# jyf588/transformer-inertial-poser

Measured on AMD Instinct MI355X. Metric: IMU frames/sec (whole node), seq_len=40 batch=256/GPU, higher is better.
Workload: dtype f32

## Files before the change

transformer-inertial-poser_amd/csrc/tip_attention.h:

```cpp
#pragma once
#include <hip/hip_runtime.h>

#include "tip_layernorm.h"

namespace tip {

typedef float f32x4_att __attribute__((ext_vector_type(4)));

template <int LDC, int LDV, bool DROP = false, int R0 = 0, int R1 = 3>
__device__ __forceinline__ void attention_head_mfma(float* Qc, float* Kc, const float* Vt, int c0, int lane, int row_limit = 48,
                                                    unsigned dkey = 0, unsigned thresh = 0, float dscale = 1.f,
                                                    unsigned long long bh = 0, int T = 0) {
    constexpr int RB = 3;
    const int l15 = lane & 15, lg = lane >> 4;
    float4 qf[RB], kf[RB];
#pragma unroll
    for (int r = 0; r < R1; ++r) {
        qf[r] = *reinterpret_cast<const float4*>(Qc + (r * 16 + l15) * LDC + c0 + lg * 4);
        kf[r] = *reinterpret_cast<const float4*>(Kc + (r * 16 + l15) * LDC + c0 + lg * 4);
    }
    f32x4_att S[RB][RB];
#pragma unroll
    for (int r = R0; r < R1; ++r)
#pragma unroll
// ... 66 lines not shown
        for (int e = 0; e < 4; ++e) {
            const float inv = __shfl(rsum[r], lg * 4 + e, 64);
            if (r * 16 + lg * 4 + e < row_limit) Qc[(r * 16 + lg * 4 + e) * LDC + c0 + l15] = o[e] * inv;
        }
    }
}

template <int LDC, bool TRAIN = false, bool STATS = true>
__device__ __forceinline__ void attention_head_regs(const f32x4_att (&qt)[3], const f32x4_att (&kt)[3], const f32x4_att (&v)[3],
                                                    float* Oc, int c0, int lane, int row_limit = 48, float* ast = nullptr,
                                                    unsigned long long bh = 0, int T = 0, unsigned long long seed = 0,
                                                    unsigned site = 0, unsigned thresh = 0, float dscale = 1.f) {
    constexpr int RB = 3;
    const int l15 = lane & 15, lg = lane >> 4;
    f32x4_att S[RB][RB];
#pragma unroll
    for (int r = 0; r < RB; ++r)
#pragma unroll
        for (int cb = 0; cb <= r; ++cb) {
            f32x4_att t = {0.f, 0.f, 0.f, 0.f};
#pragma unroll
            for (int e = 0; e < 4; ++e) t = __builtin_amdgcn_mfma_f32_16x16x4f32(kt[cb][e], qt[r][e], t, 0, 0, 0);
            S[r][cb] = t;
        }
    float mx[RB], rsum[RB];
#pragma unroll
    for (int r = 0; r < RB; ++r) {
        float m = -INFINITY;
#pragma unroll
        for (int e = 0; e < 4; ++e) {
            if (lg * 4 + e <= l15) m = fmaxf(m, S[r][r][e]);
#pragma unroll
            for (int cb = 0; cb < r; ++cb) m = fmaxf(m, S[r][cb][e]);
        }
        mx[r] = m;
    }
#pragma unroll
    for (int r = 0; r < RB; ++r) mx[r] = lg4_max(mx[r]);
#pragma unroll
    for (int r = 0; r < RB; ++r) {
        float sm = 0.f;
#pragma unroll
        for (int e = 0; e < 4; ++e) {
#pragma unroll
            for (int cb = 0; cb < r; ++cb) {
                const float p = __expf(S[r][cb][e] - mx[r]);
                S[r][cb][e] = p;
                sm += p;
            }
            const float pd = (lg * 4 + e <= l15) ? __expf(S[r][r][e] - mx[r]) : 0.f;
            S[r][r][e] = pd;
            sm += pd;
        }
        rsum[r] = sm;
    }
#pragma unroll
    for (int r = 0; r < RB; ++r) rsum[r] = lg4_sum(rsum[r]);
#pragma unroll
    for (int r = 0; r < RB; ++r) rsum[r] = 1.0f / rsum[r];
    if (TRAIN) {
        const unsigned dkey = tip_drop_key_s(seed, site);
        const __amdgpu_buffer_rsrc_t ars = tip_rows_buffer(ast + bh * T * 2, T * 8);
#pragma unroll
        for (int r = 0; r < RB; ++r) {
            const int q = r * 16 + l15;
            const ln_u32x2 mr = {__float_as_uint(mx[r]), __float_as_uint(rsum[r])};
            if (STATS) __builtin_amdgcn_raw_buffer_store_b64(mr, ars, lg == 0 ? q * 8 : T * 8, 0, 0);
            if (thresh) {
                const unsigned pb = (unsigned)((bh * T + q) * T);
#pragma unroll
                for (int cb = 0; cb <= r; ++cb)
#pragma unroll
                    for (int e = 0; e < 4; ++e)
                        S[r][cb][e] = tip_drop_hash_k(dkey, pb + cb * 16 + lg * 4 + e) >= thresh ? S[r][cb][e] * dscale : 0.f;
            }
        }
    }
#pragma unroll
    for (int r = 0; r < RB; ++r) {
        f32x4_att o = {0.f, 0.f, 0.f, 0.f};
#pragma unroll
        for (int kb = 0; kb <= r; ++kb)
#pragma unroll
            for (int e = 0; e < 4; ++e) o = __builtin_amdgcn_mfma_f32_16x16x4f32(S[r][kb][e], v[kb][e], o, 0, 0, 0);
#pragma unroll
        for (int e = 0; e < 4; ++e) {
            const float inv = __shfl(rsum[r], lg * 4 + e, 64);
            if (r * 16 + lg * 4 + e < row_limit) Oc[(r * 16 + lg * 4 + e) * LDC + c0 + l15] = o[e] * inv;
        }
    }
}

}
```

transformer-inertial-poser_amd/csrc/tip_fused.hip:

```cpp
#include <stdlib.h>
#include <string.h>

#include "tip_internal.h"
#include "tip_attention.h"
#include "tip_layernorm.h"

namespace tip {

typedef float f32x4 __attribute__((ext_vector_type(4)));

namespace fz {
constexpr int D = 256, H = 16, DH = 16, F = 1024, RP = 48, RB = 3, TMAX = 40, R = 512;
constexpr int KIN = 224;
constexpr int LDX = D + 8;
constexpr int LDC = 128 + 4;
constexpr int LDV = RP + 4;
constexpr int LDU = KIN + 8;
constexpr int X_FLOATS = RP * LDX;
constexpr int C_FLOATS = 2 * RP * LDC + 128 * LDV;
constexpr int LDS_BYTES = (X_FLOATS + C_FLOATS) * 4;
constexpr int THREADS = 512;
constexpr size_t IN_W = 0;
constexpr size_t IN_B = IN_W + (size_t)D * KIN;
constexpr size_t LAYER0 = IN_B + D;
// ... 65 lines not shown
        memcpy(L + G1, lw[8], sizeof(float) * D);
        memcpy(L + BE1, lw[9], sizeof(float) * D);
        memcpy(L + G2, lw[10], sizeof(float) * D);
        memcpy(L + BE2, lw[11], sizeof(float) * D);
    }
    if (fused_has_rnn_ih(d)) {
        const float* const* tw = t + 2 + 12 * d.L;
        float* I = dst + fused_ih_off(d);
        pack_frag(I, tw[0], R, D, D, nullptr, 1.f, 0);
        for (int i = 0; i < R; ++i) I[(size_t)R * D + i] = tw[2][i] + tw[3][i];
    }
}

static PackOp mk_op(const float* src, size_t dst, int N, int K, int src_rows, int src_cols, int frag) {
    PackOp o;
    o.src = src; o.src2 = nullptr; o.dst_off = dst; o.N = N; o.K = K; o.src_rows = src_rows; o.src_cols = src_cols; o.frag = frag;
    o.shuffle_h = 0; o.shuffle_dh = 0; o.z0 = 0; o.z1 = 0; o.scale_rows = 0; o.scale = 1.f; o.transpose = 0;
    return o;
}

void fused_pack_ops(const Dims& d, const float* const* t, size_t base, std::vector<PackOp>& ops) {
    using namespace fz;
    {
        PackOp o = mk_op(t[0], base + IN_W, D, KIN, D, d.In, 1);
        o.shuffle_h = H; o.shuffle_dh = DH;
        o.z0 = d.n_imu_total + d.rootv0; o.z1 = d.n_imu_total + d.rootv1;
        ops.push_back(o);
        PackOp b = mk_op(t[1], base + IN_B, D, 1, D, 1, 0);
        b.shuffle_h = H; b.shuffle_dh = DH;
        ops.push_back(b);
    }
    for (int l = 0; l < d.L; ++l) {
        const float* const* lw = t + 2 + 12 * l;
        const size_t L = base + LAYER0 + (size_t)l * LAYER_FLOATS;
        PackOp q = mk_op(lw[0], L + QKV_W, 3 * D, D, 3 * D, D, 1);
        q.scale = 0.25f; q.scale_rows = D;
        ops.push_back(q);
        PackOp qb = mk_op(lw[1], L + QKV_B, 3 * D, 1, 3 * D, 1, 0);
        qb.scale = 0.25f; qb.scale_rows = D;
        ops.push_back(qb);
        ops.push_back(mk_op(lw[2], L + WO_W, D, D, D, D, 1));
        ops.push_back(mk_op(lw[3], L + WO_B, D, 1, D, 1, 0));
        ops.push_back(mk_op(lw[4], L + W1_W, F, D, F, D, 1));
        ops.push_back(mk_op(lw[5], L + W1_B, F, 1, F, 1, 0));
        ops.push_back(mk_op(lw[6], L + W2_W, D, F, D, F, 1));
        ops.push_back(mk_op(lw[7], L + W2_B, D, 1, D, 1, 0));
        ops.push_back(mk_op(lw[8], L + G1, D, 1, D, 1, 0));
        ops.push_back(mk_op(lw[9], L + BE1, D, 1, D, 1, 0));
        ops.push_back(mk_op(lw[10], L + G2, D, 1, D, 1, 0));
        ops.push_back(mk_op(lw[11], L + BE2, D, 1, D, 1, 0));
    }
    if (fused_has_rnn_ih(d)) {
        const float* const* tw = t + 2 + 12 * d.L;
        const size_t I = base + fused_ih_off(d);
        ops.push_back(mk_op(tw[0], I, R, D, R, D, 1));
        PackOp b = mk_op(tw[2], I + (size_t)R * D, R, 1, R, 1, 0);
        b.src2 = tw[3];
        ops.push_back(b);
    }
}

__device__ __forceinline__ float wsum(float v) { return wave64_sum(v); }

template <int NBW, int SWAPN = 0>
__device__ __forceinline__ void mfma_block(f32x4 (&acc)[fz::RB][NBW], const float4 (&a)[fz::RB], const float4 (&w)[NBW]) {
#define TIP_MFMA_STEP(c)                                                                                             \
    _Pragma("unroll") for (int r = 0; r < fz::RB; ++r) _Pragma("unroll") for (int n = 0; n < NBW; ++n)                \
        acc[r][n] = n < SWAPN ? __builtin_amdgcn_mfma_f32_16x16x4f32(w[n].c, a[r].c, acc[r][n], 0, 0, 0)              \
                              : __builtin_amdgcn_mfma_f32_16x16x4f32(a[r].c, w[n].c, acc[r][n], 0, 0, 0);
    TIP_MFMA_STEP(x)
    TIP_MFMA_STEP(y)
    TIP_MFMA_STEP(z)
    TIP_MFMA_STEP(w)
#undef TIP_MFMA_STEP
}

typedef unsigned int u32x4 __attribute__((ext_vector_type(4)));

__device__ __forceinline__ float4 load_frag(__amdgpu_buffer_rsrc_t rsrc, int voff, int soff) {
    const f32x4 f = __builtin_bit_cast(f32x4, __builtin_amdgcn_raw_buffer_load_b128(rsrc, voff, soff, 0));
    return make_float4(f.x, f.y, f.z, f.w);
}

template <int NBW>
struct WRing {
    float4 w0[NBW], w1[NBW];
};

template <int NBW>
__device__ __forceinline__ void ring_prefetch(WRing<NBW>& g, __amdgpu_buffer_rsrc_t rsrc, int voff, int soff, int nstride_b) {
#pragma unroll
    for (int n = 0; n < NBW; ++n) {
        g.w0[n] = load_frag(rsrc, voff, soff + n * nstride_b);
        g.w1[n] = load_frag(rsrc, voff, soff + n * nstride_b + 1024);
    }
}

template <int NBW, int KB, bool NOMMA = false, int SWAPN = 0, bool PIN = true>
__device__ __forceinline__ void gemm_phase(f32x4 (&acc)[fz::RB][NBW], const float* As, int lda, __amdgpu_buffer_rsrc_t rsrc,
                                           int voff, int soff, int nstride_b, WRing<NBW>& g, int nsoff, int nnstride_b) {
    static_assert(KB % 2 == 0, "k-blocks are processed in pairs");
    float4 a0[fz::RB], a1[fz::RB];
#pragma unroll
    for (int r = 0; r < fz::RB; ++r) a0[r] = *reinterpret_cast<const float4*>(As + r * 16 * lda);
#pragma unroll 1
    for (int kb = 0; kb < KB; kb += 2) {
        const bool last = kb + 2 >= KB;
        const int o = last ? nsoff : soff + (kb + 2) * 1024;
        const int st = last ? nnstride_b : nstride_b;
#pragma unroll
        for (int r = 0; r < fz::RB; ++r) a1[r] = *reinterpret_cast<const float4*>(As + r * 16 * lda + (kb + 1) * 16);
        if (!NOMMA) mfma_block<NBW, SWAPN>(acc, a0, g.w0);
        else { asm volatile("" :: "v"(a0[0].x), "v"(g.w0[0].x)); }
#pragma unroll
        for (int n = 0; n < NBW; ++n) g.w0[n] = load_frag(rsrc, voff, o + n * st);
        if (PIN) __builtin_amdgcn_sched_barrier(0);
#pragma unroll
        for (int r = 0; r < fz::RB; ++r) a0[r] = *reinterpret_cast<const float4*>(As + r * 16 * lda + (kb + 2) * 16);
        if (!NOMMA) mfma_block<NBW, SWAPN>(acc, a1, g.w1);
        else { asm volatile("" :: "v"(a1[0].x), "v"(g.w1[0].x)); }
#pragma unroll
        for (int n = 0; n < NBW; ++n) g.w1[n] = load_frag(rsrc, voff, o + n * st + 1024);
        if (PIN) __builtin_amdgcn_sched_barrier(0);
    }
}

template <int NBW>
__device__ __forceinline__ void zero_acc(f32x4 (&acc)[fz::RB][NBW]) {
#pragma unroll
    for (int r = 0; r < fz::RB; ++r)
#pragma unroll
        for (int n = 0; n < NBW; ++n) acc[r][n] = (f32x4){0.f, 0.f, 0.f, 0.f};
}

__device__ __forceinline__ int opaque(int v) {
    asm volatile("" : "+v"(v));
    return v;
}

__device__ __forceinline__ void rows_to_hbm(const float* lds, int ld, int cols, float* dst, int dst_ld, int T, int tid) {
    const int c4n = cols >> 2;
    for (int i = tid; i < T * c4n; i += fz::THREADS) {
        const int r = i / c4n, c4 = i - r * c4n;
        __builtin_nontemporal_store(*reinterpret_cast<const f32x4*>(lds + r * ld + c4 * 4), reinterpret_cast<f32x4*>(dst + (size_t)r * dst_ld + c4 * 4));
    }
}

template <int COLS>
__device__ __forceinline__ void rows_to_hbm_fixed(const float* lds, int ld, float* dst, int dst_ld, int T, int tid) {
    constexpr int C4 = COLS / 4, NP = (40 * C4 + fz::THREADS - 1) / fz::THREADS;
    static_assert((NP * fz::THREADS + C4 - 1) / C4 <= fz::RP, "the passes stay inside the LDS tile's rows");
    const __amdgpu_buffer_rsrc_t rs = tip_rows_buffer(dst, T * dst_ld * 4);
#pragma unroll
    for (int j = 0; j < NP; ++j) {
        const int i = tid + j * fz::THREADS, r = i / C4, c4 = i - r * C4;
        const f32x4 v = *reinterpret_cast<const f32x4*>(lds + r * ld + c4 * 4);
        __builtin_amdgcn_raw_buffer_store_b128(__builtin_bit_cast(ln_u32x4, v), rs, (r * dst_ld + c4 * 4) * 4, 0, kTipNT);
    }
}

template <bool FIXED>
__device__ __forceinline__ void hidden_to_hbm(const float* lds, int ld, float* dst, int dst_ld, unsigned* gb, int f, int T, int tid) {
    typedef unsigned u32x4 __attribute__((ext_vector_type(4)));
    const int lane = tid & 63;
    if (FIXED) {
        const __amdgpu_buffer_rsrc_t rs = tip_rows_buffer(dst, T * dst_ld * 4);
// ... 438 lines not shown
    unsigned* __restrict__ hall_sentinel, int B, int T, int NI, int S, int L, int wbytes, int ih_off_b, FusedEncArgs<LIVE> tr) {
    using namespace fz;
    using namespace fzh;
    extern __shared__ __attribute__((aligned(16))) float smem[];
    float* X = smem;
    float* C = smem + X_FLOATS;
    const int tid = threadIdx.x, lane = tid & 63;
    const int wave = __builtin_amdgcn_readfirstlane(tid >> 6);
    const int l15 = lane & 15, lg = lane >> 4;
    const __amdgpu_buffer_rsrc_t rsrc = __builtin_amdgcn_make_buffer_rsrc(const_cast<float*>(wts), 0, wbytes, 0x00020000);
    const int voff = lane * 16;
    auto am = [&](int ld) { return l15 * ld + lg * 4; };
    auto at = [&](int ld) { return (TAIL0 + (lane & 3)) * ld + lg * 4; };
    constexpr bool DR = TR || LIVE;
    const LiveArgs lv = live_args_of(tr);
    unsigned long long dseed = tr.seed, sseed = 0;
    if (LIVE) {
        sseed = lv.state_seed;
        if (lv.seeds) { dseed = lv.seeds[0]; sseed = lv.seeds[1]; }
    }
    const unsigned mkey = LIVE && lv.mthresh ? tip_drop_key_s(sseed, kStateMaskSite) : 0u;

    for (int i = tid; i < 8 * LDX; i += THREADS) X[TMAX * LDX + i] = 0.f;

    for (int win = blockIdx.x; win < B; win += gridDim.x) {
        WRing<3> g_qkv;
        {
        const int layer = -1;
        FH_STAMP(0);
        if (TRACE && tid == 0 && win == (int)blockIdx.x && blockIdx.x < 1024) g_fh_wg[2 * blockIdx.x] = __builtin_amdgcn_s_memrealtime();
        const int in_soff = (int)(IN_W * 4) + (wave * 2) * (KIN / 16) * 1024;
        WRing<2> g_in;
        ring_prefetch<2>(g_in, rsrc, voff, in_soff, (KIN / 16) * 1024);
        float* U = C;
        for (int i = tid; i < RP * LDU / 4; i += THREADS) reinterpret_cast<float4*>(U)[i] = make_float4(0.f, 0.f, 0.f, 0.f);
        __syncthreads();
        {
            constexpr int NR = (TMAX + 7) / 8;
            float vi[NR][2], vs[NR][3], vk[NR][3];
            const float* kmb = keep_mask ? keep_mask : x_s;
#pragma unroll
            for (int j = 0; j < NR; ++j) {
                const int r = wave + 8 * j;
                const int rc = r < T ? r : T - 1;
                const float* xi = x_imu + ((size_t)win * T + rc) * NI;
                const float* xs = x_s + ((size_t)win * T + rc) * S;
                const float* km = kmb + ((size_t)win * T + rc) * S;
#pragma unroll
                for (int q = 0; q < 2; ++q) vi[j][q] = xi[lane + 64 * q < NI ? lane + 64 * q : NI - 1];
#pragma unroll
                for (int q = 0; q < 3; ++q) {
                    const int c = lane + 64 * q < S ? lane + 64 * q : S - 1;
                    vs[j][q] = xs[c];
                    vk[j][q] = km[c];
                }
            }
            float* pu_i = U + wave * LDU + lane;
            float* pu_s = pu_i + NI;
#pragma unroll
            for (int j = 0; j < NR; ++j) {
                if (wave + 8 * j < T) {
#pragma unroll
                    for (int q = 0; q < 2; ++q)
                        if (lane + 64 * q < NI) pu_i[8 * j * LDU + 64 * q] = vi[j][q];
#pragma unroll
                    for (int q = 0; q < 3; ++q)
                        if (lane + 64 * q < S) {
                            float v = vs[j][q];
                            if (v != v) v = 0.f;
                            if (keep_mask) v = v * vk[j][q] * keep_scale;
                            else if (LIVE && lv.mthresh)
                                v = v * (tip_drop_hash_k(mkey, ((unsigned)win * (unsigned)T + (unsigned)(wave + 8 * j)) * (unsigned)S + (unsigned)(lane + 64 * q)) >= lv.mthresh ? 1.f : 0.f) * keep_scale;
                            pu_s[8 * j * LDU + 64 * q] = v;
                        }
                }
            }
        }
        __syncthreads();
        FH_STAMP(1);
        if (TR && tr.u) rows_to_hbm_fixed<KIN>(U, LDU, tr.sv + (size_t)tr.u * 64 + (size_t)win * T * KIN, KIN, T, opaque(tid));
        {
            f32x4 acc[RBM][2], acct[RBT][2];
            zero_acc_h<2>(acc, acct);
            gemm_phase_h<2, KIN / 16, 0, TR>(acc, acct, U + am(LDU), U + at(LDU), LDU, rsrc, voff, in_soff, (KIN / 16) * 1024, g_in, in_soff,
                                      (KIN / 16) * 1024);
            ring_prefetch<3>(g_qkv, rsrc, voff, (int)(LAYER0 * 4) + (int)(QKV_W * 4) + wave * 16 * 1024, 16 * 16 * 1024);
#pragma unroll
            for (int n = 0; n < 2; ++n) {
                const int col = (wave * 2 + n) * 16 + l15;
                const float bv = wts[IN_B + col];
#pragma unroll
                for (int r = 0; r < RBM; ++r)
#pragma unroll
                    for (int e = 0; e < 4; ++e) X[(r * 16 + lg * 4 + e) * LDX + col] = acc[r][n][e] + bv;
#pragma unroll
                for (int r = 0; r < RBT; ++r) X[(TAIL0 + 4 * r + lg) * LDX + col] = tail_reduce(acct[r][n], lg) + bv;
            }
        }
        __syncthreads();
        FH_STAMP(2);
        }
        const size_t grow0 = (size_t)win * T;
        if (TR) rows_to_hbm_fixed<D>(X, LDX, tr.sv + (size_t)tr.x0 * 64 + grow0 * D, D, T, opaque(tid));
#pragma unroll 1
        for (int layer = 0; layer < L; ++layer) {
            FH_STAMP(8);
            const float* LW = wts + LAYER0 + (size_t)layer * LAYER_FLOATS;
            const int lbase = (int)((LAYER0 + (size_t)layer * LAYER_FLOATS) * 4);
            float* svl = TR ? tr.sv + (size_t)layer * tr.layer_stride * 64 : nullptr;
            const unsigned dk1 = DR ? tip_drop_key_s(dseed, (unsigned)(layer * 4 + 1)) : 0u;
            const unsigned dk2 = DR ? tip_drop_key_s(dseed, (unsigned)(layer * 4 + 2)) : 0u;
            const unsigned dk3 = DR ? tip_drop_key_s(dseed, (unsigned)(layer * 4 + 3)) : 0u;
            float bvo[2], bv2[2];
#pragma unroll
            for (int n = 0; n < 2; ++n) {
                bvo[n] = LW[WO_B + (wave * 2 + n) * 16 + l15];
                bv2[n] = LW[W2_B + (wave * 2 + n) * 16 + l15];
            }
            WRing<2> g_o, g_f;
            float* Oc = C;
#pragma unroll 1
            for (int c = 0; c < 2; ++c) {
                const int head = c * 8 + wave;
                f32x4 acc[RBM][3], acct[RBT][3];
                zero_acc_h<3>(acc, acct);
                const int qsoff = lbase + (int)(QKV_W * 4) + head * 16 * 1024;
                const int nxt = c == 0 ? qsoff + 8 * 16 * 1024 : qsoff;
                gemm_phase_h<3, 16, 2, TR>(acc, acct, X + am(LDX), X + at(LDX), LDX, rsrc, voff, qsoff, 16 * 16 * 1024, g_qkv, nxt,
                                       16 * 16 * 1024);
                if (c == 1)
                    ring_prefetch<2>(g_o, rsrc, voff, lbase + (int)(WO_W * 4) + (wave * 2) * 16 * 1024, 16 * 1024);
                const f32x4 bq = *reinterpret_cast<const f32x4*>(LW + QKV_B + head * 16 + lg * 4);
                const f32x4 bk = *reinterpret_cast<const f32x4*>(LW + QKV_B + D + head * 16 + lg * 4);
                const float bv = LW[QKV_B + 2 * D + head * 16 + l15];
                f32x4 qt[RB], kt[RB], vv[RB];
#pragma unroll
                for (int r = 0; r < RBM; ++r) {
                    qt[r] = acc[r][0] + bq;
                    kt[r] = acc[r][1] + bk;
                    vv[r] = acc[r][2] + bv;
                }
                vv[2] = tail_gather_v(acct[0][2], acct[1][2], lg);
                if (lg < 2) vv[2] += bv;
                {
                    constexpr int SLD = 20;
                    float* scr = C + RP * LDX + wave * (2 * 8 * SLD);
                    const float bqp = LW[QKV_B + head * 16 + l15], bkp = LW[QKV_B + D + head * 16 + l15];
#pragma unroll
                    for (int rb = 0; rb < RBT; ++rb) {
                        scr[(4 * rb + lg) * SLD + l15] = tail_reduce(acct[rb][0], lg) + bqp;
                        scr[8 * SLD + (4 * rb + lg) * SLD + l15] = tail_reduce(acct[rb][1], lg) + bkp;
                    }
                    __builtin_amdgcn_fence(__ATOMIC_RELEASE, "wavefront");
                    __builtin_amdgcn_wave_barrier();
                    __builtin_amdgcn_fence(__ATOMIC_ACQUIRE, "wavefront");
                    const f32x4 z = {0.f, 0.f, 0.f, 0.f};
                    qt[2] = l15 < 8 ? *reinterpret_cast<const f32x4*>(scr + l15 * SLD + lg * 4) : z;
                    kt[2] = l15 < 8 ? *reinterpret_cast<const f32x4*>(scr + 8 * SLD + l15 * SLD + lg * 4) : z;
                    __builtin_amdgcn_wave_barrier();
                }
                FH_STAMP(9 + 4 * c);
                if (TR) {
                    const __amdgpu_buffer_rsrc_t qp_rs = tip_rows_buffer(svl + (size_t)tr.qkv * 64 + grow0 * (3 * D), T * 3 * D * 4);
                    const int lo = opaque(lane), l15o = lo & 15, lgo = lo >> 4;
#pragma unroll
                    for (int r = 0; r < RB; ++r) {
                        const int qo = ((r * 16 + l15o) * (3 * D) + head * 16 + lgo * 4) * 4;
                        __builtin_amdgcn_raw_buffer_store_b128(__builtin_bit_cast(u32x4, qt[r] * 4.0f), qp_rs, qo, 0, kTipNT);
                        __builtin_amdgcn_raw_buffer_store_b128(__builtin_bit_cast(u32x4, kt[r]), qp_rs, qo + D * 4, 0, kTipNT);
#pragma unroll
                        for (int e = 0; e < 4; ++e)
                            __builtin_amdgcn_raw_buffer_store_b32(__float_as_uint(vv[r][e]), qp_rs,
                                                                  ((r * 16 + lgo * 4 + e) * (3 * D) + 2 * D + head * 16 + l15o) * 4, 0, kTipNT);
                    }
                    attention_head_regs<LDX, true>(qt, kt, vv, Oc, head * 16, lo, TMAX, svl + (size_t)tr.ast * 64,
                                                   (unsigned long long)win * H + head, T, tr.seed, (unsigned)(layer * 4 + 0), tr.thresh,
                                                   tr.scale);
                } else if (LIVE) {
                    attention_head_regs<LDX, true, false>(qt, kt, vv, Oc, head * 16, opaque(lane), TMAX, nullptr, (unsigned long long)win * H + head, T,
                                                          dseed, (unsigned)(layer * 4 + 0), tr.thresh, tr.scale);
                } else {
                    attention_head_regs<LDX>(qt, kt, vv, Oc, head * 16, lane, TMAX);
                }
                FH_STAMP(10 + 4 * c);
            }
            __syncthreads();
            FH_STAMP(15);
            if (TR) rows_to_hbm_fixed<D>(Oc, LDX, svl + (size_t)tr.att * 64 + grow0 * D, D, T, opaque(tid));
            ring_prefetch<2>(g_f, rsrc, voff, lbase + (int)(W1_W * 4) + (wave * 2) * 16 * 1024, 16 * 1024);
            f32x4 acc_o[RBM][2], acc_ot[RBT][2];
            zero_acc_h<2>(acc_o, acc_ot);
            {
                const int osoff = lbase + (int)(WO_W * 4) + (wave * 2) * 16 * 1024;
                gemm_phase_h<2, 16, 0, TR>(acc_o, acc_ot, Oc + am(LDX), Oc + at(LDX), LDX, rsrc, voff, osoff, 16 * 1024, g_o, osoff, 16 * 1024);
            }
            __syncthreads();
            FH_STAMP(16);
            float xr[2][RBM][4], xt[2][RBT];
#pragma unroll
            for (int n = 0; n < 2; ++n) {
                const int col = (wave * 2 + n) * 16 + l15;
#pragma unroll
                for (int r = 0; r < RBM; ++r)
#pragma unroll
                    for (int e = 0; e < 4; ++e) xr[n][r][e] = X[(r * 16 + lg * 4 + e) * LDX + col];
#pragma unroll
                for (int r = 0; r < RBT; ++r) xt[n][r] = X[(TAIL0 + 4 * r + lg) * LDX + col];
            }
#pragma unroll
            for (int n = 0; n < 2; ++n) {
                const int col = (wave * 2 + n) * 16 + l15;
                const float bv = bvo[n];
                    const int hl = LIVE ? opaque(lane) : lane, hlg = LIVE ? hl >> 4 : lg, hcol = LIVE ? (wave * 2 + n) * 16 + (hl & 15) : col;
#pragma unroll
                for (int r = 0; r < RBM; ++r)
#pragma unroll
                    for (int e = 0; e < 4; ++e) {
                        float v = acc_o[r][n][e] + bv;
                        if (DR && tr.thresh)
                            v = tip_drop_hash_k(dk1, (grow0 + r * 16 + hlg * 4 + e) * D + hcol) >= tr.thresh ? v * tr.scale : 0.f;
                        X[(r * 16 + lg * 4 + e) * LDX + col] = xr[n][r][e] + v;
                    }
#pragma unroll
                for (int r = 0; r < RBT; ++r) {
                    float v = tail_reduce(acc_ot[r][n], lg) + bv;
                    if (DR && tr.thresh)
                        v = tip_drop_hash_k(dk1, (grow0 + TAIL0 + 4 * r + hlg) * D + hcol) >= tr.thresh ? v * tr.scale : 0.f;
                    X[(TAIL0 + 4 * r + lg) * LDX + col] = xt[n][r] + v;
                }
            }
            __syncthreads();
            FH_STAMP(17);
            if (TR)
                layernorm_rows16<fz::TMAX, fz::LDX, true>(X, LW + G1, LW + BE1, wave, opaque(lane), svl + (size_t)tr.z1 * 64 + grow0 * D,
                                                          svl + (size_t)tr.st1 * 64 + grow0 * 2, svl + (size_t)tr.x1 * 64 + grow0 * D, T);
            else
                layernorm_rows16<fz::TMAX, fz::LDX>(X, LW + G1, LW + BE1, wave, lane);
            __syncthreads();
            FH_STAMP(18);
            float* Hc = C;
            f32x4 acc_f[RBM][2], acc_ft[RBT][2];
            zero_acc_h<2>(acc_f, acc_ft);
#pragma unroll 1
            for (int f = 0; f < 4; ++f) {
                {
                    f32x4 acc[RBM][2], acct[RBT][2];
                    zero_acc_h<2>(acc, acct);
                    const int nb0 = f * 16 + wave * 2;
                    const int w1off = lbase + (int)(W1_W * 4) + nb0 * 16 * 1024;
                    const int w2off = lbase + (int)(W2_W * 4) + ((wave * 2) * 64 + f * 16) * 1024;
                    float bv1[2];
#pragma unroll
                    for (int n = 0; n < 2; ++n) bv1[n] = LW[W1_B + f * 256 + (wave * 2 + n) * 16 + l15];
                    gemm_phase_h<2, 16, 0, TR>(acc, acct, X + am(LDX), X + at(LDX), LDX, rsrc, voff, w1off, 16 * 1024, g_f, w2off, 64 * 1024);
#pragma unroll
                    for (int n = 0; n < 2; ++n) {
                        const int col = (wave * 2 + n) * 16 + l15;
                        const float bv = bv1[n];
                    const int hl = LIVE ? opaque(lane) : lane, hlg = LIVE ? hl >> 4 : lg, hcol = LIVE ? (wave * 2 + n) * 16 + (hl & 15) : col;
#pragma unroll
                        for (int r = 0; r < RBM; ++r)
#pragma unroll
                            for (int e = 0; e < 4; ++e) {
                                float v = fmaxf(acc[r][n][e] + bv, 0.f);
                                if (DR && tr.thresh)
                                    v = tip_drop_hash_k(dk2, (grow0 + r * 16 + hlg * 4 + e) * F + f * 256 + hcol) >= tr.thresh ? v * tr.scale : 0.f;
                                Hc[(r * 16 + lg * 4 + e) * LDX + col] = v;
                            }
#pragma unroll
                        for (int r = 0; r < RBT; ++r) {
                            float v = fmaxf(tail_reduce(acct[r][n], lg) + bv, 0.f);
                            if (DR && tr.thresh)
                                v = tip_drop_hash_k(dk2, (grow0 + TAIL0 + 4 * r + hlg) * F + f * 256 + hcol) >= tr.thresh ? v * tr.scale : 0.f;
                            Hc[(TAIL0 + 4 * r + lg) * LDX + col] = v;
                        }
                    }
                }
                FH_STAMP(19 + 3 * f);
                __syncthreads();
                FH_STAMP(20 + 3 * f);
                if (TR)
                    hidden_to_hbm<true>(Hc, LDX, svl + (size_t)tr.hid * 64 + grow0 * F + f * 256, F,
                                  reinterpret_cast<unsigned*>(svl + (size_t)tr.hid * 64 + (size_t)B * T * F) + grow0 * 32, f, T, opaque(tid));
                {
                    const int w2off = lbase + (int)(W2_W * 4) + ((wave * 2) * 64 + f * 16) * 1024;
                    const int nxt = f < 3 ? lbase + (int)(W1_W * 4) + ((f + 1) * 16 + wave * 2) * 16 * 1024 : w2off;
                    gemm_phase_h<2, 16, 0, TR>(acc_f, acc_ft, Hc + am(LDX), Hc + at(LDX), LDX, rsrc, voff, w2off, 64 * 1024, g_f, nxt,
                                        f < 3 ? 16 * 1024 : 64 * 1024);
                }
                __syncthreads();
                FH_STAMP(21 + 3 * f);
            }
            if (layer + 1 < L)
                ring_prefetch<3>(g_qkv, rsrc, voff, lbase + (int)(LAYER_FLOATS * 4) + (int)(QKV_W * 4) + wave * 16 * 1024, 16 * 16 * 1024);
#pragma unroll
            for (int n = 0; n < 2; ++n) {
                const int col = (wave * 2 + n) * 16 + l15;
#pragma unroll
                for (int r = 0; r < RBM; ++r)
#pragma unroll
                    for (int e = 0; e < 4; ++e) xr[n][r][e] = X[(r * 16 + lg * 4 + e) * LDX + col];
#pragma unroll
                for (int r = 0; r < RBT; ++r) xt[n][r] = X[(TAIL0 + 4 * r + lg) * LDX + col];
            }
#pragma unroll
            for (int n = 0; n < 2; ++n) {
                const int col = (wave * 2 + n) * 16 + l15;
                const float bv = bv2[n];
                    const int hl = LIVE ? opaque(lane) : lane, hlg = LIVE ? hl >> 4 : lg, hcol = LIVE ? (wave * 2 + n) * 16 + (hl & 15) : col;
#pragma unroll
                for (int r = 0; r < RBM; ++r)
#pragma unroll
                    for (int e = 0; e < 4; ++e) {
                        float v = acc_f[r][n][e] + bv;
                        if (DR && tr.thresh)
                            v = tip_drop_hash_k(dk3, (grow0 + r * 16 + hlg * 4 + e) * D + hcol) >= tr.thresh ? v * tr.scale : 0.f;
                        X[(r * 16 + lg * 4 + e) * LDX + col] = xr[n][r][e] + v;
                    }
#pragma unroll
                for (int r = 0; r < RBT; ++r) {
                    float v = tail_reduce(acc_ft[r][n], lg) + bv;
                    if (DR && tr.thresh)
                        v = tip_drop_hash_k(dk3, (grow0 + TAIL0 + 4 * r + hlg) * D + hcol) >= tr.thresh ? v * tr.scale : 0.f;
                    X[(TAIL0 + 4 * r + lg) * LDX + col] = xt[n][r] + v;
                }
            }
            __syncthreads();
            FH_STAMP(31);
            if (TR)
                layernorm_rows16<fz::TMAX, fz::LDX, true>(X, LW + G2, LW + BE2, wave, opaque(lane), svl + (size_t)tr.z2 * 64 + grow0 * D,
                                                          svl + (size_t)tr.st2 * 64 + grow0 * 2, svl + (size_t)tr.xo * 64 + grow0 * D, T);
            else
                layernorm_rows16<fz::TMAX, fz::LDX>(X, LW + G2, LW + BE2, wave, lane);
            __syncthreads();
            FH_STAMP(32);
        }
        { const int layer = -1; FH_STAMP(40); }
        if (ih_out) {
            f32x4 acc[RBM][4], acct[RBT][4];
            zero_acc_h<4>(acc, acct);
            const int isoff = ih_off_b + (wave * 4) * 16 * 1024;
            WRing<4> g_ih;
            ring_prefetch<4>(g_ih, rsrc, voff, isoff, 16 * 1024);
            gemm_phase_h<4, 16, 4, TR>(acc, acct, X + am(LDX), X + at(LDX), LDX, rsrc, voff, isoff, 16 * 1024, g_ih, isoff, 16 * 1024);
            const __amdgpu_buffer_rsrc_t io_rs = __builtin_amdgcn_make_buffer_rsrc(ih_out + (size_t)win * T * R, 0, T * R * 4, 0x00020000);
            const int lo = opaque(lane), l15o = lo & 15, lgo = lo >> 4;
            float bvs[4];
            f32x4 bv4s[4];
#pragma unroll
            for (int n = 0; n < 4; ++n) {
                bvs[n] = wts[ih_off_b / 4 + R * D + (wave * 4 + n) * 16 + l15o];
                bv4s[n] = *reinterpret_cast<const f32x4*>(wts + ih_off_b / 4 + R * D + (wave * 4 + n) * 16 + lgo * 4);
            }
#pragma unroll
            for (int n = 0; n < 4; ++n) {
                const int col = (wave * 4 + n) * 16 + l15o;
#pragma unroll
                for (int r = 0; r < RBM; ++r) {
                    const int row = r * 16 + l15o;
                    __builtin_amdgcn_raw_buffer_store_b128(__builtin_bit_cast(u32x4, acc[r][n] + bv4s[n]), io_rs, (row * R + (wave * 4 + n) * 16 + lgo * 4) * 4, 0, 0);
                }
#pragma unroll
                for (int r = 0; r < RBT; ++r) {
                    const float v = tail_reduce(acct[r][n], lg) + bvs[n];
                    const int row = TAIL0 + 4 * r + lgo;
                    __builtin_amdgcn_raw_buffer_store_b32(__float_as_uint(v), io_rs, (row * R + col) * 4, 0, 0);
                }
            }
        }
        if (hall_sentinel) {
            uint4* hp = reinterpret_cast<uint4*>(hall_sentinel + (size_t)win * T * R);
            for (int i = opaque(tid); i < T * (R / 4); i += THREADS) hp[i] = make_uint4(0xFFFFFFFFu, 0xFFFFFFFFu, 0xFFFFFFFFu, 0xFFFFFFFFu);
        }
        if (xout) {
            float* out = xout + (size_t)win * T * D;
            for (int i = tid; i < T * (D / 4); i += THREADS) {
                const int r = i / (D / 4), c4 = i - r * (D / 4);
                *reinterpret_cast<float4*>(out + (size_t)r * D + c4 * 4) = *reinterpret_cast<const float4*>(X + r * LDX + c4 * 4);
            }
        }
        __syncthreads();
        { const int layer = -1; FH_STAMP(41); }
        if (TRACE && tid == 0 && blockIdx.x < 1024) g_fh_wg[2 * blockIdx.x + 1] = __builtin_amdgcn_s_memrealtime();
    }
}
#undef FH_STAMP

hipError_t launch_fused_encoder_h(const Dims& d, const float* fused_w, const float* x_imu, const float* x_s,
                                  const float* keep_mask, float keep_scale, float* xout, float* ih_out, float* hall_sentinel,
                                  int B, int T, int num_cus, hipStream_t s) {
    if (B <= 0) return hipSuccess;
    static PerDeviceFlag attr_flag; bool& attr_set = attr_flag.cur();
    if (!attr_set) {
        for (const void* f : {reinterpret_cast<const void*>(fused_encoder_h_kernel<false, false>), reinterpret_cast<const void*>(fused_encoder_h_kernel<true, false>)}) {
            hipError_t e = hipFuncSetAttribute(f, hipFuncAttributeMaxDynamicSharedMemorySize, fz::LDS_BYTES);
            if (e != hipSuccess) return e;
        }
        attr_set = true;
    }
    static int trace = -1;
    if (trace < 0) trace = tip_env("TIP_FUSEDH_TRACE") ? 1 : 0;
// ... 744 lines not shown
```

Before: 412,300.

## Transpose MFMA accumulator layout for vectorized LDS epilogue stores and buffer-loaded biases

Swaps the MFMA operand order in the attention P·V product and in the main GEMM phases (template arg 0 to 2). Each lane then holds four consecutive columns of one row, so outputs, residual reads and writes can use 128-bit LDS accesses instead of four strided scalar ones. Biases are now fetched as float4 and scalar values through buffer loads, and the dropout hash indices are remapped to match the transposed layout. The intent is fewer LDS instructions and fewer bank conflicts in the epilogues. The cost is extra bias loads per phase and a risk of indexing mismatches in the tail and dropout paths.

Measured after the change: 414,300 (median of 6 runs). About the same (+0.5%).

```diff
diff --git a/transformer-inertial-poser_amd/csrc/tip_attention.h b/transformer-inertial-poser_amd/csrc/tip_attention.h
--- a/transformer-inertial-poser_amd/csrc/tip_attention.h
+++ b/transformer-inertial-poser_amd/csrc/tip_attention.h
@@ -172,12 +172,8 @@
 #pragma unroll
         for (int kb = 0; kb <= r; ++kb)
 #pragma unroll
-            for (int e = 0; e < 4; ++e) o = __builtin_amdgcn_mfma_f32_16x16x4f32(S[r][kb][e], v[kb][e], o, 0, 0, 0);
-#pragma unroll
-        for (int e = 0; e < 4; ++e) {
-            const float inv = __shfl(rsum[r], lg * 4 + e, 64);
-            if (r * 16 + lg * 4 + e < row_limit) Oc[(r * 16 + lg * 4 + e) * LDC + c0 + l15] = o[e] * inv;
-        }
+            for (int e = 0; e < 4; ++e) o = __builtin_amdgcn_mfma_f32_16x16x4f32(v[kb][e], S[r][kb][e], o, 0, 0, 0);
+        if (r * 16 + l15 < row_limit) *reinterpret_cast<f32x4_att*>(Oc + (r * 16 + l15) * LDC + c0 + lg * 4) = o * rsum[r];
     }
 }
 
diff --git a/transformer-inertial-poser_amd/csrc/tip_fused.hip b/transformer-inertial-poser_amd/csrc/tip_fused.hip
--- a/transformer-inertial-poser_amd/csrc/tip_fused.hip
+++ b/transformer-inertial-poser_amd/csrc/tip_fused.hip
@@ -171,6 +171,13 @@
     return make_float4(f.x, f.y, f.z, f.w);
 }
 
+__device__ __forceinline__ f32x4 load_bias4(__amdgpu_buffer_rsrc_t rsrc, int voff, int soff) {
+    return __builtin_bit_cast(f32x4, __builtin_amdgcn_raw_buffer_load_b128(rsrc, voff, soff, 0));
+}
+__device__ __forceinline__ float load_bias1(__amdgpu_buffer_rsrc_t rsrc, int voff, int soff) {
+    return __uint_as_float(__builtin_amdgcn_raw_buffer_load_b32(rsrc, voff, soff, 0));
+}
+
 template <int NBW>
 struct WRing {
     float4 w0[NBW], w1[NBW];
@@ -775,17 +782,16 @@
         {
             f32x4 acc[RBM][2], acct[RBT][2];
             zero_acc_h<2>(acc, acct);
-            gemm_phase_h<2, KIN / 16, 0, TR>(acc, acct, U + am(LDU), U + at(LDU), LDU, rsrc, voff, in_soff, (KIN / 16) * 1024, g_in, in_soff,
+            gemm_phase_h<2, KIN / 16, 2, TR>(acc, acct, U + am(LDU), U + at(LDU), LDU, rsrc, voff, in_soff, (KIN / 16) * 1024, g_in, in_soff,
                                       (KIN / 16) * 1024);
             ring_prefetch<3>(g_qkv, rsrc, voff, (int)(LAYER0 * 4) + (int)(QKV_W * 4) + wave * 16 * 1024, 16 * 16 * 1024);
 #pragma unroll
             for (int n = 0; n < 2; ++n) {
-                const int col = (wave * 2 + n) * 16 + l15;
-                const float bv = wts[IN_B + col];
-#pragma unroll
-                for (int r = 0; r < RBM; ++r)
-#pragma unroll
-                    for (int e = 0; e < 4; ++e) X[(r * 16 + lg * 4 + e) * LDX + col] = acc[r][n][e] + bv;
+                const int cb = (wave * 2 + n) * 16, col = cb + l15;
+                const f32x4 bv4 = load_bias4(rsrc, lg * 16, (int)(IN_B * 4) + cb * 4);
+                const float bv = load_bias1(rsrc, l15 * 4, (int)(IN_B * 4) + cb * 4);
+#pragma unroll
+                for (int r = 0; r < RBM; ++r) *reinterpret_cast<f32x4*>(X + am(LDX) + r * 16 * LDX + cb) = acc[r][n] + bv4;
 #pragma unroll
                 for (int r = 0; r < RBT; ++r) X[(TAIL0 + 4 * r + lg) * LDX + col] = tail_reduce(acct[r][n], lg) + bv;
             }
@@ -805,11 +811,7 @@
             const unsigned dk2 = DR ? tip_drop_key_s(dseed, (unsigned)(layer * 4 + 2)) : 0u;
             const unsigned dk3 = DR ? tip_drop_key_s(dseed, (unsigned)(layer * 4 + 3)) : 0u;
             float bvo[2], bv2[2];
-#pragma unroll
-            for (int n = 0; n < 2; ++n) {
-                bvo[n] = LW[WO_B + (wave * 2 + n) * 16 + l15];
-                bv2[n] = LW[W2_B + (wave * 2 + n) * 16 + l15];
-            }
+            f32x4 bvo4[2], bv24[2];
             WRing<2> g_o, g_f;
             float* Oc = C;
 #pragma unroll 1
@@ -883,37 +885,42 @@
             ring_prefetch<2>(g_f, rsrc, voff, lbase + (int)(W1_W * 4) + (wave * 2) * 16 * 1024, 16 * 1024);
             f32x4 acc_o[RBM][2], acc_ot[RBT][2];
             zero_acc_h<2>(acc_o, acc_ot);
+#pragma unroll
+            for (int n = 0; n < 2; ++n) {
+                bvo[n] = load_bias1(rsrc, l15 * 4, lbase + (int)(WO_B * 4) + (wave * 2 + n) * 64);
+                bvo4[n] = load_bias4(rsrc, lg * 16, lbase + (int)(WO_B * 4) + (wave * 2 + n) * 64);
+            }
             {
                 const int osoff = lbase + (int)(WO_W * 4) + (wave * 2) * 16 * 1024;
-                gemm_phase_h<2, 16, 0, TR>(acc_o, acc_ot, Oc + am(LDX), Oc + at(LDX), LDX, rsrc, voff, osoff, 16 * 1024, g_o, osoff, 16 * 1024);
+                gemm_phase_h<2, 16, 2, TR>(acc_o, acc_ot, Oc + am(LDX), Oc + at(LDX), LDX, rsrc, voff, osoff, 16 * 1024, g_o, osoff, 16 * 1024);
             }
             __syncthreads();
             FH_STAMP(16);
-            float xr[2][RBM][4], xt[2][RBT];
+            f32x4 xr[2][RBM];
+            float xt[2][RBT];
 #pragma unroll
             for (int n = 0; n < 2; ++n) {
-                const int col = (wave * 2 + n) * 16 + l15;
-#pragma unroll
-                for (int r = 0; r < RBM; ++r)
-#pragma unroll
-                    for (int e = 0; e < 4; ++e) xr[n][r][e] = X[(r * 16 + lg * 4 + e) * LDX + col];
+                const int cb = (wave * 2 + n) * 16, col = cb + l15;
+#pragma unroll
+                for (int r = 0; r < RBM; ++r) xr[n][r] = *reinterpret_cast<const f32x4*>(X + am(LDX) + r * 16 * LDX + cb);
 #pragma unroll
                 for (int r = 0; r < RBT; ++r) xt[n][r] = X[(TAIL0 + 4 * r + lg) * LDX + col];
             }
 #pragma unroll
             for (int n = 0; n < 2; ++n) {
-                const int col = (wave * 2 + n) * 16 + l15;
+                const int cb = (wave * 2 + n) * 16, col = cb + l15;
                 const float bv = bvo[n];
-                    const int hl = LIVE ? opaque(lane) : lane, hlg = LIVE ? hl >> 4 : lg, hcol = LIVE ? (wave * 2 + n) * 16 + (hl & 15) : col;
-#pragma unroll
-                for (int r = 0; r < RBM; ++r)
-#pragma unroll
-                    for (int e = 0; e < 4; ++e) {
-                        float v = acc_o[r][n][e] + bv;
-                        if (DR && tr.thresh)
-                            v = tip_drop_hash_k(dk1, (grow0 + r * 16 + hlg * 4 + e) * D + hcol) >= tr.thresh ? v * tr.scale : 0.f;
-                        X[(r * 16 + lg * 4 + e) * LDX + col] = xr[n][r][e] + v;
-                    }
+                    const int hl = LIVE ? opaque(lane) : lane, hlg = LIVE ? hl >> 4 : lg, hl15 = LIVE ? hl & 15 : l15, hcol = cb + hl15;
+#pragma unroll
+                for (int r = 0; r < RBM; ++r) {
+                    f32x4 v = acc_o[r][n] + bvo4[n];
+                    if (DR && tr.thresh) {
+#pragma unroll
+                        for (int e = 0; e < 4; ++e)
+                            v[e] = tip_drop_hash_k(dk1, (grow0 + r * 16 + hl15) * D + cb + hlg * 4 + e) >= tr.thresh ? v[e] * tr.scale : 0.f;
+                    }
+                    *reinterpret_cast<f32x4*>(X + am(LDX) + r * 16 * LDX + cb) = xr[n][r] + v;
+                }
 #pragma unroll
                 for (int r = 0; r < RBT; ++r) {
                     float v = tail_reduce(acc_ot[r][n], lg) + bv;
@@ -943,23 +950,29 @@
                     const int w1off = lbase + (int)(W1_W * 4) + nb0 * 16 * 1024;
                     const int w2off = lbase + (int)(W2_W * 4) + ((wave * 2) * 64 + f * 16) * 1024;
                     float bv1[2];
-#pragma unroll
-                    for (int n = 0; n < 2; ++n) bv1[n] = LW[W1_B + f * 256 + (wave * 2 + n) * 16 + l15];
-                    gemm_phase_h<2, 16, 0, TR>(acc, acct, X + am(LDX), X + at(LDX), LDX, rsrc, voff, w1off, 16 * 1024, g_f, w2off, 64 * 1024);
+                    f32x4 bv14[2];
 #pragma unroll
                     for (int n = 0; n < 2; ++n) {
-                        const int col = (wave * 2 + n) * 16 + l15;
+                        bv1[n] = load_bias1(rsrc, l15 * 4, lbase + (int)(W1_B * 4) + f * 1024 + (wave * 2 + n) * 64);
+                        bv14[n] = load_bias4(rsrc, lg * 16, lbase + (int)(W1_B * 4) + f * 1024 + (wave * 2 + n) * 64);
+                    }
+                    gemm_phase_h<2, 16, 2, TR>(acc, acct, X + am(LDX), X + at(LDX), LDX, rsrc, voff, w1off, 16 * 1024, g_f, w2off, 64 * 1024);
+#pragma unroll
+                    for (int n = 0; n < 2; ++n) {
+                        const int cb = (wave * 2 + n) * 16, col = cb + l15;
                         const float bv = bv1[n];
-                    const int hl = LIVE ? opaque(lane) : lane, hlg = LIVE ? hl >> 4 : lg, hcol = LIVE ? (wave * 2 + n) * 16 + (hl & 15) : col;
-#pragma unroll
-                        for (int r = 0; r < RBM; ++r)
+                    const int hl = LIVE ? opaque(lane) : lane, hlg = LIVE ? hl >> 4 : lg, hl15 = LIVE ? hl & 15 : l15, hcol = cb + hl15;
+#pragma unroll
+                        for (int r = 0; r < RBM; ++r) {
+                            f32x4 v = acc[r][n] + bv14[n];
 #pragma unroll
                             for (int e = 0; e < 4; ++e) {
-                                float v = fmaxf(acc[r][n][e] + bv, 0.f);
+                                v[e] = fmaxf(v[e], 0.f);
                                 if (DR && tr.thresh)
-                                    v = tip_drop_hash_k(dk2, (grow0 + r * 16 + hlg * 4 + e) * F + f * 256 + hcol) >= tr.thresh ? v * tr.scale : 0.f;
-                                Hc[(r * 16 + lg * 4 + e) * LDX + col] = v;
+                                    v[e] = tip_drop_hash_k(dk2, (grow0 + r * 16 + hl15) * F + f * 256 + cb + hlg * 4 + e) >= tr.thresh ? v[e] * tr.scale : 0.f;
                             }
+                            *reinterpret_cast<f32x4*>(Hc + am(LDX) + r * 16 * LDX + cb) = v;
+                        }
 #pragma unroll
                         for (int r = 0; r < RBT; ++r) {
                             float v = fmaxf(tail_reduce(acct[r][n], lg) + bv, 0.f);
@@ -978,7 +991,12 @@
                 {
                     const int w2off = lbase + (int)(W2_W * 4) + ((wave * 2) * 64 + f * 16) * 1024;
                     const int nxt = f < 3 ? lbase + (int)(W1_W * 4) + ((f + 1) * 16 + wave * 2) * 16 * 1024 : w2off;
-                    gemm_phase_h<2, 16, 0, TR>(acc_f, acc_ft, Hc + am(LDX), Hc + at(LDX), LDX, rsrc, voff, w2off, 64 * 1024, g_f, nxt,
+#pragma unroll
+                    for (int n = 0; n < 2; ++n) {
+                        bv2[n] = load_bias1(rsrc, l15 * 4, lbase + (int)(W2_B * 4) + (wave * 2 + n) * 64);
+                        bv24[n] = load_bias4(rsrc, lg * 16, lbase + (int)(W2_B * 4) + (wave * 2 + n) * 64);
+                    }
+                    gemm_phase_h<2, 16, 2, TR>(acc_f, acc_ft, Hc + am(LDX), Hc + at(LDX), LDX, rsrc, voff, w2off, 64 * 1024, g_f, nxt,
                                         f < 3 ? 16 * 1024 : 64 * 1024);
                 }
                 __syncthreads();
@@ -988,28 +1006,27 @@
                 ring_prefetch<3>(g_qkv, rsrc, voff, lbase + (int)(LAYER_FLOATS * 4) + (int)(QKV_W * 4) + wave * 16 * 1024, 16 * 16 * 1024);
 #pragma unroll
             for (int n = 0; n < 2; ++n) {
-                const int col = (wave * 2 + n) * 16 + l15;
-#pragma unroll
-                for (int r = 0; r < RBM; ++r)
-#pragma unroll
-                    for (int e = 0; e < 4; ++e) xr[n][r][e] = X[(r * 16 + lg * 4 + e) * LDX + col];
+                const int cb = (wave * 2 + n) * 16, col = cb + l15;
+#pragma unroll
+                for (int r = 0; r < RBM; ++r) xr[n][r] = *reinterpret_cast<const f32x4*>(X + am(LDX) + r * 16 * LDX + cb);
 #pragma unroll
                 for (int r = 0; r < RBT; ++r) xt[n][r] = X[(TAIL0 + 4 * r + lg) * LDX + col];
             }
 #pragma unroll
             for (int n = 0; n < 2; ++n) {
-                const int col = (wave * 2 + n) * 16 + l15;
+                const int cb = (wave * 2 + n) * 16, col = cb + l15;
                 const float bv = bv2[n];
-                    const int hl = LIVE ? opaque(lane) : lane, hlg = LIVE ? hl >> 4 : lg, hcol = LIVE ? (wave * 2 + n) * 16 + (hl & 15) : col;
-#pragma unroll
-                for (int r = 0; r < RBM; ++r)
-#pragma unroll
-                    for (int e = 0; e < 4; ++e) {
-                        float v = acc_f[r][n][e] + bv;
-                        if (DR && tr.thresh)
-                            v = tip_drop_hash_k(dk3, (grow0 + r * 16 + hlg * 4 + e) * D + hcol) >= tr.thresh ? v * tr.scale : 0.f;
-                        X[(r * 16 + lg * 4 + e) * LDX + col] = xr[n][r][e] + v;
-                    }
+                    const int hl = LIVE ? opaque(lane) : lane, hlg = LIVE ? hl >> 4 : lg, hl15 = LIVE ? hl & 15 : l15, hcol = cb + hl15;
+#pragma unroll
+                for (int r = 0; r < RBM; ++r) {
+                    f32x4 v = acc_f[r][n] + bv24[n];
+                    if (DR && tr.thresh) {
+#pragma unroll
+                        for (int e = 0; e < 4; ++e)
+                            v[e] = tip_drop_hash_k(dk3, (grow0 + r * 16 + hl15) * D + cb + hlg * 4 + e) >= tr.thresh ? v[e] * tr.scale : 0.f;
+                    }
+                    *reinterpret_cast<f32x4*>(X + am(LDX) + r * 16 * LDX + cb) = xr[n][r] + v;
+                }
 #pragma unroll
                 for (int r = 0; r < RBT; ++r) {
                     float v = tail_reduce(acc_ft[r][n], lg) + bv;
```
